# BCAM-CFD/RigidMultiblobsWall

Measured on AMD Instinct MI355X. Metric: RPY-wall M.f matvecs/sec (single_wall_mobility_trans_times_force, N_blobs=10000), higher is better.
Workload: dtype f64

## Files before the change

### include/rmb_mobility.h

```cpp
#ifndef RMB_MOBILITY_H
#define RMB_MOBILITY_H

#include <stddef.h>

#ifdef __cplusplus
extern "C" {
#endif

typedef struct rmb_ctx rmb_ctx;

enum rmb_status {
  RMB_OK = 0,
  RMB_ERR_ARG = -1,
  RMB_ERR_STATE = -2,
  RMB_ERR_HIP = -3,
  RMB_ERR_NO_DEVICE = -4
};

enum rmb_kind { RMB_TT = 0, RMB_TR = 1, RMB_RT = 2, RMB_RR = 3, RMB_TT_TR = 4, RMB_TT_FREE_SURFACE = 5 };

const char* rmb_version(void);
const char* rmb_last_error(void);
int rmb_device_count(void);

// ... 119 lines not shown
                             double body_repulsion_strength, double body_debye_length, double kT, double* energy_dev,
                             int* accepted_dev);
int rmb_one_blob_force_device(rmb_ctx* ctx, long n, const double* r_dev, double blob_radius, double weight, double eps_wall,
                              double debye_wall, int accumulate, double* out_dev);
int rmb_blob_blob_force_pairshard_device(rmb_ctx* ctx, double repulsion_strength, double debye_length,
                                         double blob_radius, double* out_dev, long shard, long nshards);
int rmb_blob_blob_force_radii(rmb_ctx* ctx, const double* radii, double repulsion_strength, double debye_length,
                              double* out);
int rmb_blob_blob_force_radii_device(rmb_ctx* ctx, const double* radii_dev, double repulsion_strength,
                                     double debye_length, double* out_dev);

int rmb_timing_collect(rmb_ctx* ctx, double* ms, int max_n);
int rmb_timing_reset(rmb_ctx* ctx);
int rmb_ubench_fp64_issue(rmb_ctx* ctx, int launches, double* g_wave_instr_per_s);
int rmb_wave_clock_collect(rmb_ctx* ctx, long long* stamps, long max_waves);
int rmb_last_host_timing(rmb_ctx* ctx, double* us4);
int rmb_last_launch(rmb_ctx* ctx, long* tiles, long* chunks, long* workgroups);
int rmb_ctx_synchronize(rmb_ctx* ctx);

int rmb_default_ctx_set_option(const char* key, long value);
int rmb_default_ctx_set_device(int device);

typedef struct rmb_multi rmb_multi;
int rmb_multi_create(const int* devices, int n_devices, rmb_multi** engine);
int rmb_multi_destroy(rmb_multi* engine);
int rmb_multi_n_shards(rmb_multi* engine);
int rmb_multi_shard_ctx(rmb_multi* engine, int shard, rmb_ctx** ctx);
int rmb_multi_set_stream(rmb_multi* engine, void* hip_stream);
int rmb_multi_set_option(rmb_multi* engine, const char* key, long value);
int rmb_multi_get_option(rmb_multi* engine, const char* key, long* value);
// ... 61 lines not shown
```

### rigidmultiblobswall_amd/_lib.py

```python
import ctypes
import os

_HERE = os.path.dirname(os.path.abspath(__file__))
DIAGNOSTICS = os.environ.get("RMB_DIAGNOSTICS", "0") not in ("", "0")
LIB_PATH = os.path.join(_HERE, "librmb_mobility_diag.so" if DIAGNOSTICS else "librmb_mobility.so")

_dp = ctypes.POINTER(ctypes.c_double)
_vp = ctypes.c_void_p
_lp = ctypes.POINTER(ctypes.c_long)

KIND_TT, KIND_TR, KIND_RT, KIND_RR, KIND_TT_TR, KIND_TT_FREE = 0, 1, 2, 3, 4, 5
OP_VELOCITY_FROM_FORCE_TORQUE, OP_GRAND, OP_FORCE_COLUMN, OP_TT_MULTI, OP_TR_MULTI, OP_RT_MULTI, OP_RR_MULTI = range(7)
OPS = {"velocity_from_force_torque": (OP_VELOCITY_FROM_FORCE_TORQUE, 2, 1), "grand": (OP_GRAND, 2, 2),
       "force_column": (OP_FORCE_COLUMN, 1, 2), "tt_multi": (OP_TT_MULTI, None, None), "tr_multi": (OP_TR_MULTI, None, None),
       "rt_multi": (OP_RT_MULTI, None, None), "rr_multi": (OP_RR_MULTI, None, None)}
KINDS = {"tt": KIND_TT, "tr": KIND_TR, "rt": KIND_RT, "rr": KIND_RR, "tt_tr": KIND_TT_TR, "tt_free": KIND_TT_FREE}

SYMBOLS = {
    "rmb_version": (ctypes.c_char_p, []),
    "rmb_last_error": (ctypes.c_char_p, []),
    "rmb_device_count": (ctypes.c_int, []),
    "rmb_ctx_create": (ctypes.c_int, [ctypes.c_int, ctypes.POINTER(_vp)]),
    "rmb_ctx_destroy": (ctypes.c_int, [_vp]),
    "rmb_ctx_set_stream": (ctypes.c_int, [_vp, _vp]),
# ... 63 lines not shown
                                                    _vp, _vp] + [ctypes.c_double] * 6 + [ctypes.c_int, ctypes.c_double, ctypes.c_double, _vp]),
    "rmb_mcmc_sweep_bb_device": (ctypes.c_int, [_vp, ctypes.c_long, ctypes.c_long, ctypes.c_long, _vp, _vp, _vp, _vp, _vp, _vp, _vp, ctypes.c_double,
                                               _vp] + [ctypes.c_double] * 6 + [ctypes.c_int, ctypes.c_double, ctypes.c_double, ctypes.c_double,
                                                                               _vp, _vp]),
    "rmb_potential_oneshot": (ctypes.c_int, [ctypes.c_long, _vp, _vp] + [ctypes.c_double] * 6 + [ctypes.c_int, _vp]),
    "rmb_one_blob_force_device": (ctypes.c_int, [_vp, ctypes.c_long, _vp, ctypes.c_double, ctypes.c_double, ctypes.c_double, ctypes.c_double,
                                                ctypes.c_int, _vp]),
    "rmb_blob_blob_force_pairshard_device": (ctypes.c_int, [_vp, ctypes.c_double, ctypes.c_double, ctypes.c_double, _vp,
                                                            ctypes.c_long, ctypes.c_long]),
    "rmb_blob_blob_force_radii": (ctypes.c_int, [_vp, _vp, ctypes.c_double, ctypes.c_double, _vp]),
    "rmb_blob_blob_force_radii_device": (ctypes.c_int, [_vp, _vp, ctypes.c_double, ctypes.c_double, _vp]),
    "rmb_timing_collect": (ctypes.c_int, [_vp, _dp, ctypes.c_int]),
    "rmb_timing_reset": (ctypes.c_int, [_vp]),
    "rmb_ubench_fp64_issue": (ctypes.c_int, [_vp, ctypes.c_int, _dp]),
    "rmb_wave_clock_collect": (ctypes.c_int, [_vp, _vp, ctypes.c_long]),
    "rmb_last_host_timing": (ctypes.c_int, [_vp, _dp]),
    "rmb_last_launch": (ctypes.c_int, [_vp, _lp, _lp, _lp]),
    "rmb_ctx_synchronize": (ctypes.c_int, [_vp]),
    "rmb_default_ctx_set_option": (ctypes.c_int, [ctypes.c_char_p, ctypes.c_long]),
    "rmb_default_ctx_set_device": (ctypes.c_int, [ctypes.c_int]),
    "rmb_multi_create": (ctypes.c_int, [ctypes.POINTER(ctypes.c_int), ctypes.c_int, ctypes.POINTER(_vp)]),
    "rmb_multi_destroy": (ctypes.c_int, [_vp]),
    "rmb_multi_n_shards": (ctypes.c_int, [_vp]),
    "rmb_multi_shard_ctx": (ctypes.c_int, [_vp, ctypes.c_int, ctypes.POINTER(_vp)]),
    "rmb_multi_set_stream": (ctypes.c_int, [_vp, _vp]),
    "rmb_multi_set_option": (ctypes.c_int, [_vp, ctypes.c_char_p, ctypes.c_long]),
    "rmb_multi_get_option": (ctypes.c_int, [_vp, ctypes.c_char_p, _lp]),
    "rmb_multi_set_positions": (ctypes.c_int, [_vp, _vp, ctypes.c_long, ctypes.c_double, _vp, ctypes.c_int]),
    "rmb_multi_set_positions_device": (ctypes.c_int, [_vp, _vp, ctypes.c_long, ctypes.c_double, _vp, ctypes.c_int]),
    "rmb_multi_matvec": (ctypes.c_int, [_vp, ctypes.c_int, ctypes.c_int, _vp, _vp, ctypes.c_double, _vp]),
# ... 86 lines not shown
```

### rigidmultiblobswall_amd/context.py

```python
import ctypes

import numpy as np

from . import _lib


def _as_f64(x, n3=None):
  x = np.ascontiguousarray(x, dtype=np.float64).reshape(-1)
  if n3 is not None and x.size != n3:
    raise ValueError("expected %d values, got %d" % (n3, x.size))
  return x


def _ptr(x):
  return ctypes.c_void_p(x.ctypes.data)


POTENTIAL_FORMS = {"soft": 0, "yukawa": 1}
VAN_HOVE_PLANES = {"xyz": 0, "xy": 1}


class MobilityContext(object):

  def __init__(self, device=0):
# ... 745 lines not shown

  def timing_collect(self, max_n=8192):
    buf = (ctypes.c_double * max_n)()
    n = self._lib.rmb_timing_collect(self._h, buf, max_n)
    if n < 0:
      _lib.check(n)
    return np.array(buf[:n])

  def wave_clock_collect(self, max_waves=8192):
    buf = np.zeros((max_waves, 2), dtype=np.int64)
    n = self._lib.rmb_wave_clock_collect(self._h, ctypes.c_void_p(buf.ctypes.data), max_waves)
    if n < 0:
      _lib.check(n)
    return buf[:n]

  def ubench_fp64_issue(self, launches=40):
    out = ctypes.c_double()
    self._follow_torch_stream()
    _lib.check(self._lib.rmb_ubench_fp64_issue(self._h, int(launches), ctypes.byref(out)))
    return float(out.value)

  def last_host_timing(self):
    buf = (ctypes.c_double * 4)()
    _lib.check(self._lib.rmb_last_host_timing(self._h, buf))
    return dict(upload_us=buf[0], launch_us=buf[1], wait_and_download_us=buf[2], c_call_us=buf[3])

  def timing_reset(self):
    _lib.check(self._lib.rmb_timing_reset(self._h))

  def last_launch(self):
# ... 54 lines not shown
```

### rigidmultiblobswall_amd/csrc/rmb_context.hip

```cpp
#include "rmb_internal.h"

#include <cstdint>
#include <cstdio>
#include <cstdlib>
#include <cstring>

namespace rmbi {

namespace { thread_local std::string g_err; }

int fail(int code, const std::string& msg) {
  g_err = msg;
  return code;
}

int DevBuf::reserve(size_t bytes) {
  if (bytes <= cap) return 0;
  if (p) { (void)hipFree(p); p = nullptr; cap = 0; }
  size_t want = bytes + bytes / 8 + 256;
  hipError_t e = hipMalloc(&p, want);
  if (e != hipSuccess) { p = nullptr; return fail(RMB_ERR_HIP, std::string("hipMalloc: ") + hipGetErrorString(e)); }
  cap = want;
  return 0;
}
// ... 83 lines not shown
    {"det_workspace_mb", &rmb_ctx::opt_det_workspace_mb, CLAMP, 1, kNoCap},
    {"sym_wps", &rmb_ctx::opt_sym_wps}, {"sym_pin", &rmb_ctx::opt_sym_pin},
    {"free_surface", &rmb_ctx::opt_free_surface, BOOLEAN}, {"free_surface_rotation", &rmb_ctx::opt_free_surface_rotation, BOOLEAN},
    {"precision", &rmb_ctx::opt_precision, ONE_OF, 32, 64, 64, "precision must be 32 or 64"},
    {"force_precision", &rmb_ctx::opt_force_precision, ONE_OF, 0, 32, 64, "force_precision must be 0 (follow \"precision\"), 32 or 64"},
    {"force_cull", &rmb_ctx::opt_force_cull, BOOLEAN}, {"force_sort", &rmb_ctx::opt_force_sort, BOOLEAN},
    {"potential_resort", &rmb_ctx::opt_potential_resort, CLAMP, 1, kNoCap},
    {"sym_fine_steps", &rmb_ctx::opt_sym_fine_steps, CLAMP, 0, kNoCap},
    {"sym_coop", &rmb_ctx::opt_sym_coop, ONE_OF, 0, 1, 2, "sym_coop must be 0 (never), 1 (launches below one resident round) or 2 (always)"},
    {"sym_chunk_steps", &rmb_ctx::opt_sym_chunk_steps, CLAMP, 0, kNoCap}, {"sym_two_targets", &rmb_ctx::opt_sym_two_targets, CLAMP, 0, 2},
    {"host_zero_copy_in", &rmb_ctx::opt_host_zero_copy_in, BOOLEAN}, {"gmres_fuse_pc", &rmb_ctx::opt_gmres_fuse_pc, BOOLEAN}, {"gmres_fuse_dots", &rmb_ctx::opt_gmres_fuse_dots, BOOLEAN},
    {"krylov_low_sync", &rmb_ctx::opt_krylov_low_sync, BOOLEAN}, {"lanczos_fuse_finish", &rmb_ctx::opt_lanczos_fuse_finish, BOOLEAN},
    {"host_zero_copy", &rmb_ctx::opt_host_zero_copy, CLAMP, 0, kNoCap},
    {"sym_order", &rmb_ctx::opt_sym_order, BOOLEAN}, {"sym_xcd", &rmb_ctx::opt_sym_xcd, BOOLEAN},
    {"sym_oversub", &rmb_ctx::opt_sym_oversub, CLAMP, 1, kNoCap}, {"sym_min_steps", &rmb_ctx::opt_sym_min_steps, CLAMP, 1, kNoCap},
    {"wave_clock", &rmb_ctx::opt_wave_clock, AS_GIVEN, 0, 0, 0, nullptr, true}, {"skip_pairs", &rmb_ctx::opt_skip_pairs, AS_GIVEN, 0, 0, 0, nullptr, true},
};

const Option* find_option(const char* key) {
  for (const Option& o : kOptions)
    if (!strcmp(key, o.key)) return &o;
  return nullptr;
}
}

}

using namespace rmbi;

extern "C" {

const char* rmb_version(void) { return "rmb_mobility 0.1 (gfx950)"; }
const char* rmb_last_error(void) { return rmbi::g_err.c_str(); }

int rmb_device_count(void) {
  int n = 0;
  if (hipGetDeviceCount(&n) != hipSuccess) return 0;
// ... 6 lines not shown
  hipError_t e = hipGetDeviceCount(&n);
  if (e != hipSuccess || n == 0)
    return fail(RMB_ERR_NO_DEVICE, std::string("no HIP device visible (") + hipGetErrorString(e) + ")");
  if (device == -1) {
    device = default_device();
    if (device < 0) return fail(RMB_ERR_ARG, "RMB_DEVICE must be a non-negative device index");
  }
  if (device < 0 || device >= n) return fail(RMB_ERR_ARG, "device index out of range");
  RMB_HIP(hipSetDevice(device));
  hipDeviceProp_t prop;
  RMB_HIP(hipGetDeviceProperties(&prop, device));
  rmb_ctx* c = new rmb_ctx();
  c->device = device;
  if (prop.multiProcessorCount > 0) c->n_cu = prop.multiProcessorCount;
  if (prop.maxSharedMemoryPerMultiProcessor > 0) c->lds_per_cu = prop.maxSharedMemoryPerMultiProcessor;
  *out = c;
  return 0;
}

int rmb_ctx_destroy(rmb_ctx* c) {
  if (!c) return 0;
  (void)hipSetDevice(c->device);
  (void)hipStreamSynchronize(c->stream);
  rmbi::gmres_release(c);
  for_each_buffer(*c, [](DevBuf& b) { b.release(); });
  c->host_out.release();
  c->host_in.release();
  if (c->stream_switch) (void)hipEventDestroy(c->stream_switch);
  for (auto e : c->ev0) (void)hipEventDestroy(e);
  for (auto e : c->ev1) (void)hipEventDestroy(e);
// ... 38 lines not shown
    case CLAMP: value = value < o->a ? o->a : (value > o->b ? o->b : value); break;
    case BOOLEAN: value = value ? 1 : 0; break;
    case ONE_OF: if (value != o->a && value != o->b && value != o->c) return fail(RMB_ERR_ARG, o->refusal); break;
  }
  c->*(o->field) = value;
  if (o->field == &rmb_ctx::opt_potential_resort) c->pot_sort_age = -1;
  return 0;
}

int rmb_ctx_get_option(rmb_ctx* c, const char* key, long* value) {
  if (!c || !key || !value) return fail(RMB_ERR_ARG, "null context / key / value");
  if (!strcmp(key, "last_path")) { *value = c->last_path; return 0; }
  if (!strcmp(key, "diagnostics_build")) { *value = kDiagnosticsBuild; return 0; }
  if (!strcmp(key, "buffers_signature")) {
    unsigned long long h = 1469598103934665603ull;
    for_each_buffer(*c, [&h](const DevBuf& b) { h = (h ^ (unsigned long long)(uintptr_t)b.p) * 1099511628211ull; });
    *value = (long)(h >> 1);
    return 0;
  }
  const Option* o = find_option(key);
  if (!o) return fail(RMB_ERR_ARG, std::string("unknown option: ") + key);
  *value = c->*(o->field);
  return 0;
}

int rmb_timing_collect(rmb_ctx* c, double* ms, int max_n) {
  if (!c || !ms || max_n < 0) return fail(RMB_ERR_ARG, "bad timing_collect arguments");
  if (hipSetDevice(c->device) != hipSuccess) return fail(RMB_ERR_HIP, "hipSetDevice failed");
  if (hipStreamSynchronize(c->stream) != hipSuccess) return fail(RMB_ERR_HIP, "hipStreamSynchronize failed");
  int have = c->ev_count < kTimingRing ? c->ev_count : kTimingRing;
  if (have > max_n) have = max_n;
  for (int i = 0; i < have; ++i) {
    const int idx = (c->ev_count - have + i) % kTimingRing;
    float t = 0.f;
    if (hipEventElapsedTime(&t, c->ev0[idx], c->ev1[idx]) != hipSuccess) return fail(RMB_ERR_HIP, "hipEventElapsedTime failed");
    ms[i] = (double)t;
  }
  return have;
// ... 62 lines not shown
```

### rigidmultiblobswall_amd/csrc/rmb_internal.h

```cpp
#pragma once
#include "../../include/rmb_mobility.h"

#include <hip/hip_runtime.h>

#include <cmath>
#include <mutex>
#include <string>
#include <type_traits>
#include <vector>

#include "pair_ops.h"

namespace rmbi {

int fail(int code, const std::string& msg);

#define RMB_HIP(call)                                                                        \
  do {                                                                                       \
    hipError_t e_ = (call);                                                                  \
    if (e_ != hipSuccess)                                                                    \
      return rmbi::fail(RMB_ERR_HIP, std::string(#call) + ": " + hipGetErrorString(e_));     \
  } while (0)

struct DevBuf {
  void* p = nullptr;
  size_t cap = 0;
// ... 14 lines not shown
struct CtxBuffers {
  DevBuf pos;
  DevBuf r_stage;
  DevBuf vec, vec2, out, partial, tmp3n;
  DevBuf tile_bounds;
  DevBuf fpos, fperm, fsort_keys, fsort_vals, fsort_tmp, fsort_box;
  DevBuf pot_ws;
  DevBuf mcmc_ws;
  DevBuf msd_ws;
  DevBuf scat_ws;
  DevBuf vh_ws;
  DevBuf det_ws;
  DevBuf wave_clock;
  DevBuf krylov;
  DevBuf symbuf;
  DevBuf st[8];
};
using CB = CtxBuffers;
constexpr DevBuf CB::* kCtxBufs[] = {&CB::pos, &CB::r_stage, &CB::vec, &CB::vec2, &CB::out, &CB::partial, &CB::tmp3n, &CB::tile_bounds,
                                     &CB::fpos, &CB::fperm, &CB::fsort_keys, &CB::fsort_vals, &CB::fsort_tmp, &CB::fsort_box,
                                     &CB::pot_ws, &CB::mcmc_ws, &CB::msd_ws, &CB::scat_ws, &CB::vh_ws, &CB::det_ws, &CB::wave_clock, &CB::krylov, &CB::symbuf};
static_assert(sizeof(CtxBuffers) == (sizeof(kCtxBufs) / sizeof(kCtxBufs[0]) + 8) * sizeof(DevBuf),
              "a DevBuf of CtxBuffers is missing from kCtxBufs (or st[] changed its length)");
template <class Bufs, class F>
void for_each_buffer(Bufs& b, F f) {
  for (auto m : kCtxBufs) f(b.*m);
  for (auto& s : b.st) f(s);
}

}

struct rmb_ctx : rmbi::CtxBuffers {
  int device = 0;
  hipStream_t stream = nullptr;
  hipEvent_t stream_switch = nullptr;
  long n_cu = 256;
// ... 31 lines not shown
  long opt_potential_resort = 16;
  long opt_sym_fine_steps = 0;
  long opt_sym_coop = 1;
  long opt_sym_chunk_steps = 1024;
  long opt_sym_two_targets = 1;
  long opt_host_zero_copy_in = 1;
  long opt_gmres_fuse_pc = 1;
  long opt_gmres_fuse_dots = 1;
  long opt_krylov_low_sync = 1;
  long opt_lanczos_fuse_finish = 1;
  long opt_host_zero_copy = 768 << 10;
  long opt_sym_order = 1;
  long opt_sym_xcd = 1;
  long opt_sym_oversub = 8;
  long opt_sym_min_steps = 64;
  long opt_wave_clock = 0;
  long opt_skip_pairs = 0;
  std::vector<hipEvent_t> ev0, ev1;
  int ev_count = 0;
  long timing_launches = 0;
  int last_path = 0;
  long last_tiles = 0, last_chunks = 0, last_wgs = 0;
  double host_us[4] = {0, 0, 0, 0};
};

namespace rmbi {

int timing_begin(rmb_ctx* c, int* slot);
int timing_end(rmb_ctx* c, int slot);
int check_ready(rmb_ctx* c);
// ... 72 lines not shown
}
int plan_cull_sweep(rmb_ctx* c, const SymKernel& k, long total_steps, long* blocks, long* chunk_steps, long rounds = 0,
                    size_t dyn_lds = 0, double wg_pair_cap = 0.0, const char* who = "");
void shard_ranges(long n, long n_units, long shard, long nshards, long* step_begin, long* step_end, long* self_begin,
                  long* self_end);
int sym_accumulators(rmb_ctx* c, long n_pad);
long chunked_steps(const rmb_ctx* c, long total, long n_sched, long spw, long target);
bool sym_applies(const rmb_ctx* c);
inline double inv_length(double L) { return L > 0 ? 1.0 / L : 0.0; }

enum SymXOp { SX_TT = 0, SX_TR, SX_RT, SX_RR, SX_FUSED, SX_GRAND, SX_COLF, SX_FREE, SX_RADII,
              SX_FREE_TR, SX_FREE_RT, SX_FREE_RR, SX_FREE_FUSED, SX_FREE_GRAND, SX_FREE_COLF, SX_K2, SX_COUNT = SX_K2 + 12 };
struct SymConf { const double4* pos; long n; double L[3]; int wall; const double* extra; };
template <class A, class = void> struct HasNPad : std::false_type {};
template <class A> struct HasNPad<A, std::void_t<decltype(A::n_pad)>> : std::true_type {};
template <class A, class = void> struct HasPrefactor : std::false_type {};
template <class A> struct HasPrefactor<A, std::void_t<decltype(A::prefactor)>> : std::true_type {};
template <class Args>
void fill_sym_args(Args& a, const SymConf& cf, const rmb_ctx* c, double eta, long n_units, long shard, long nshards) {
  const long tiles = (cf.n + 63) / 64;
  long step_begin, step_end, self_begin, self_end;
  shard_ranges(cf.n, n_units, shard, nshards, &step_begin, &step_end, &self_begin, &self_end);
  a.pos = cf.pos;
  a.n = cf.n; a.n_tiles = (int)tiles;
  a.order = (int)c->opt_sym_order; a.xcd = (int)c->opt_sym_xcd;
  a.step_end = step_end;
  a.Lx = cf.L[0]; a.Ly = cf.L[1];
  a.iLx = inv_length(cf.L[0]); a.iLy = inv_length(cf.L[1]);
  if constexpr (HasNPad<Args>::value) {
    a.acc = (double*)c->symbuf.p;
    a.n_pad = 64 * tiles; a.n_units = n_units;
    a.step_begin = step_begin;
    a.Lz = cf.L[2]; a.iLz = inv_length(cf.L[2]);
  }
  if constexpr (HasPrefactor<Args>::value) {
    a.self_begin = self_begin; a.self_end = self_end;
    a.prefactor = 1.0 / (8.0 * M_PI * eta);
    a.k = make_pair_consts(c->a > 0.0 ? c->a : 1.0);
  }
}
template <class Args>
int sym_launch(rmb_ctx* c, const SymKernel& k, int path, long blocks, size_t dyn_lds, Args& a, const rmb::PairConsts& pk,
               void (*fin)(Args), long fin_blocks, long long** wave_clock = nullptr) {
  c->last_path = path; c->last_tiles = a.n_tiles; c->last_chunks = 0; c->last_wgs = blocks;
  if (wave_clock) {
    *wave_clock = nullptr;
    if (c->opt_wave_clock) {
      c->wave_clock_n = blocks * rmb::kSymWaves * (path == 4 ? 2 : 1);
      if (int rc = c->wave_clock.reserve((size_t)2 * c->wave_clock_n * sizeof(long long))) return rc;
      *wave_clock = (long long*)c->wave_clock.p;
    }
  }
  int slot;
  if (int rc = timing_begin(c, &slot)) return rc;
// ... 79 lines not shown
```

### rigidmultiblobswall_amd/csrc/rmb_sym.hip

```cpp
#include "rmb_internal.h"

#include <cmath>

#include "sym_kernels.h"
#include "sym_coop_kernels.h"
#include "sym2t_kernels.h"
#include "sym2_kernels.h"
#include "sym_force_kernels.h"
#include "sym_schedule.h"
#include "symx_kernels.h"

namespace rmbi {

namespace {
SymConf conf_of(const rmb_ctx* c) {
  return SymConf{(const double4*)c->pos.p, c->n, {c->L[0], c->L[1], c->L[2]}, c->wall, nullptr};
}
bool is_periodic(const SymConf& cf) { return cf.L[0] > 0 || cf.L[1] > 0 || cf.L[2] > 0; }

struct SymCandidates { SymKernel plain, coop, two, f32; };
struct SymChoice {
  SymKernel kernel;
  SymPlan plan;
  int path;
// ... 43 lines not shown
struct SymEntry { SymCandidates k; sym_fn fin; };
template <int KIND, bool WALL, bool PER> SymEntry make_sym_entry() {
  constexpr size_t lds = sizeof(double2) * rmb::kSymWaves * 64 * 3 + sizeof(double) * rmb::kSymWaves * 3 * 64;
  constexpr size_t coop_lds = sizeof(double2) * 64 * 3 + sizeof(double) * 2 * 3 * 64;
  SymEntry e{{sym_kernel_of<rmb::SymArgs, rmb::sym_kernel<KIND, WALL, PER>>(lds, rmb::kSymWavesPerEu),
              sym_kernel_of<rmb::SymArgs, rmb::sym_coop_kernel<KIND, WALL, PER>>(coop_lds, rmb::kSymWavesPerEu), SymKernel{}, SymKernel{}},
             rmb::sym_finalize_kernel<KIND, WALL>};
  if constexpr (!PER) e.k.two = sym_kernel_of<rmb::SymArgs, rmb::sym2t_kernel<KIND, WALL>>(lds, rmb::kSymWavesPerEu);
  return e;
}
#define RMB_SYM_ROW(K) {{make_sym_entry<K, false, false>(), make_sym_entry<K, false, true>()}, {make_sym_entry<K, true, false>(), make_sym_entry<K, true, true>()}}
SymEntry g_sym[4][2][2] = {RMB_SYM_ROW(rmb::KIND_TT), RMB_SYM_ROW(rmb::KIND_TR), RMB_SYM_ROW(rmb::KIND_RT), RMB_SYM_ROW(rmb::KIND_RR)};
#undef RMB_SYM_ROW
}

int sym_device(rmb_ctx* c, int kind, const double* v, double eta, double* out, long shard, long nshards, bool accumulate,
               bool no_finalize) {
  const SymConf cf = conf_of(c);
  const bool periodic = is_periodic(cf);
  const SymEntry& se = g_sym[kind][c->wall ? 1 : 0][periodic ? 1 : 0];
  const long n = c->n;
  if (int rc = sym_accumulators(c, 64 * ((n + 63) / 64))) return rc;
  if (periodic && no_finalize) return fail(RMB_ERR_STATE, "sym_device: no_finalize is for open boundaries (internal)");
  SymCandidates k = se.k;
  if (periodic && !c->opt_wave_clock) k.two = symx_two_periodic(SX_TT + kind, c->wall != 0);
  if (c->opt_wave_clock) k.coop = SymKernel{};
  if (c->opt_precision == 32 && kind == RMB_TT && !periodic) {
    if (c->opt_wave_clock || c->opt_skip_pairs)
      return fail(RMB_ERR_STATE, "the \"wave_clock\" / \"skip_pairs\" diagnostics exist in the fp64 kernels only: set \"precision\" = 64");
    k.f32 = sym32_tt(c->wall != 0);
  }
  SymChoice ch;
  if (int rc = choose_sym(c, k, n, shard, nshards, kCoopMaxRounds, true, &ch)) return rc;
  if (periodic && ch.path == 4) {
    const double* in[2] = {v, nullptr};
    double* outs[1] = {out};
    return symx_device(c, SX_TT + kind, in, outs, eta, 0, shard, nshards, accumulate ? 1 : 0);
  }
  rmb::SymArgs a;
  fill_sym_args(a, cf, c, eta, ch.n_units, shard, nshards);
  a.vec = v;
  a.out = out;
  a.steps_per_wave = ch.steps_per_wave;
  a.skip_pairs = (int)c->opt_skip_pairs;
  a.accumulate = accumulate ? 1 : 0;
  return sym_launch(c, ch.kernel, ch.path, ch.plan.blocks, ch.plan.dyn_lds, a, a.k, no_finalize ? nullptr : se.fin, (n + 255) / 256,
                    &a.wave_clock);
}

int sym2_device(rmb_ctx* c, const double* va, const double* vb, double eta, double* out_a, double* out_b, long shard,
                long nshards) {
  const SymConf cf = conf_of(c);
  const bool periodic = is_periodic(cf);
  const long n = c->n;
  if (int rc = sym_accumulators(c, 64 * ((n + 63) / 64))) return rc;
  typedef rmb::Sym2Args A;
  const SymKernel k = c->wall ? (periodic ? sym_kernel_of<A, rmb::sym2_kernel<true, true>>(0, rmb::kSymWavesPerEu)
                                          : sym_kernel_of<A, rmb::sym2_kernel<true, false>>(0, rmb::kSymWavesPerEu))
                              : (periodic ? sym_kernel_of<A, rmb::sym2_kernel<false, true>>(0, rmb::kSymWavesPerEu)
                                          : sym_kernel_of<A, rmb::sym2_kernel<false, false>>(0, rmb::kSymWavesPerEu));
  SymChoice ch;
  if (int rc = choose_sym(c, SymCandidates{k, SymKernel{}, SymKernel{}, SymKernel{}}, n, shard, nshards, 0, false, &ch)) return rc;
// ... 201 lines not shown
```

### rigidmultiblobswall_amd/csrc/sym2t_kernels.h

```cpp
#pragma once
#include "sym_kernels.h"
#include "sym_schedule.h"

namespace rmb {

template <int KIND, bool WALL>
__global__ __launch_bounds__(64 * kSymWaves) __attribute__((amdgpu_waves_per_eu(kSymWavesPerEu, kSymWavesPerEu))) void sym2t_kernel(const SymArgs a) {
  __shared__ double2 rec_all[kSymWaves][64 * 3];
  __shared__ double accj_all[kSymWaves][3 * 64];
  const int lane = threadIdx.x & 63;
  const int wave = __builtin_amdgcn_readfirstlane(threadIdx.x >> 6);
  double2* rec = rec_all[wave];
  double* accj = accj_all[wave];
  const char* rec_bytes = reinterpret_cast<const char*>(rec);
  constexpr bool Z2 = kSymZi2<KIND, WALL>;

  const long w = (a.xcd ? xcd_swizzle(blockIdx.x, gridDim.x) : (long)blockIdx.x) * kSymWaves + wave;
  const long long t_start = a.wave_clock ? wall_clock64() : 0;
  const long long c_start = a.wave_clock ? (long long)__builtin_readcyclecounter() : 0;
  long long c_stage = 0;
  for (long chunk = w;; chunk += (long)gridDim.x * kSymWaves) {
  long s = a.step_begin + chunk * a.steps_per_wave;
  if (s >= a.step_end) break;
  long s_end = s + a.steps_per_wave;
  if (s_end > a.step_end) s_end = a.step_end;
  int p = 0, J = 0;
  unit2_seek(a.order, s >> 6, a.n_tiles, p, J);

  int p_cur = -1;
  long i0 = 0, i1 = 0;
  bool ok0 = false, ok1 = false;
  double x0 = 0, y0 = 0, z0 = sym_height<Z2>(1.0), v0x = 0, v0y = 0, v0z = 0;
  double x1 = 0, y1 = 0, z1 = sym_height<Z2>(1.0), v1x = 0, v1y = 0, v1z = 0;
  Vec3 u0 = {0.0, 0.0, 0.0}, u1 = {0.0, 0.0, 0.0};

  auto flush_rows = [&]() {
    if (ok0) {
      __hip_atomic_fetch_add(&a.acc[i0], u0.x, __ATOMIC_RELAXED, __HIP_MEMORY_SCOPE_AGENT);
      __hip_atomic_fetch_add(&a.acc[a.n_pad + i0], u0.y, __ATOMIC_RELAXED, __HIP_MEMORY_SCOPE_AGENT);
      __hip_atomic_fetch_add(&a.acc[2 * a.n_pad + i0], u0.z, __ATOMIC_RELAXED, __HIP_MEMORY_SCOPE_AGENT);
// ... 95 lines not shown
      __builtin_amdgcn_fence(__ATOMIC_RELEASE, "wavefront");
      __builtin_amdgcn_wave_barrier();
      __builtin_amdgcn_fence(__ATOMIC_ACQUIRE, "wavefront");
      const long j = 64L * J + lane;
      if (j < a.n && !(a.skip_pairs & 2)) {
        __hip_atomic_fetch_add(&a.acc[j], accj[lane], __ATOMIC_RELAXED, __HIP_MEMORY_SCOPE_AGENT);
        __hip_atomic_fetch_add(&a.acc[a.n_pad + j], accj[64 + lane], __ATOMIC_RELAXED, __HIP_MEMORY_SCOPE_AGENT);
        __hip_atomic_fetch_add(&a.acc[2 * a.n_pad + j], accj[128 + lane], __ATOMIC_RELAXED, __HIP_MEMORY_SCOPE_AGENT);
      }
    }
    __builtin_amdgcn_wave_barrier();
    if (k1 == 64) unit2_next(a.order, a.n_tiles, p, J);
  }
  if (p_cur >= 0) flush_rows();
  }
  if (a.wave_clock && lane == 0) {
    const unsigned hw = __builtin_amdgcn_s_getreg((4) | (0 << 6) | ((16 - 1) << 11));
    const unsigned xcc = __builtin_amdgcn_s_getreg((20) | (0 << 6) | ((4 - 1) << 11));
    const long n_waves = (long)gridDim.x * kSymWaves;
    a.wave_clock[2 * w] = t_start;
    a.wave_clock[2 * w + 1] = (wall_clock64() & 0xffffffffffLL) | ((long long)(hw & 0xffff) << 40) | ((long long)(xcc & 0xf) << 56);
    a.wave_clock[2 * (n_waves + w)] = c_stage;
    a.wave_clock[2 * (n_waves + w) + 1] = (long long)__builtin_readcyclecounter() - c_start;
  }
}

}
```

### rigidmultiblobswall_amd/csrc/sym_kernels.h

```cpp
#pragma once
#include "pair_blocks.h"
#include "sym_schedule.h"

namespace rmb {

struct SymArgs {
  const double4* pos;
  const double* vec;
  double* acc;
  double* out;
  long n;
  long n_pad;
  int n_tiles;
  long n_units;
  int order;
  int xcd;
  long step_begin, step_end;
  long steps_per_wave;
  long self_begin, self_end;
  double Lx, Ly, Lz, iLx, iLy, iLz;
  double prefactor;
  int accumulate;
  int skip_pairs;
  long long* wave_clock;
  PairConsts k;
};

constexpr int kSymRecBytes = 48;

template <bool WALL, bool ACC = false, bool ZI2 = false>
__device__ __forceinline__ void pair_tt_sym(const PairConsts& k, double dx, double dy, double dz, double zi, double zj,
                                            double vix, double viy, double viz, double vjx, double vjy, double vjz,
                                            Vec3& ui, double& tx, double& ty, double& tz) {
  const Geom g = make_geom<WALL, ZI2>(dx, dy, dz, zi, zj);
  const TTc c = tt_coeffs<WALL, ZI2>(k, g, zi, zj);
  const double vi[3] = {vix, viy, viz}, vj[3] = {vjx, vjy, vjz};
  double u[3] = {ui.x, ui.y, ui.z}, t[3];
  if constexpr (ACC) { t[0] = tx; t[1] = ty; t[2] = tz; }
  tt_apply<WALL, ACC>(c, g, vi, vj, u, t);
  ui.x = u[0]; ui.y = u[1]; ui.z = u[2];
  tx = t[0]; ty = t[1]; tz = t[2];
// ... 45 lines not shown


template <int KIND, bool WALL, bool PERIODIC>
__global__ __launch_bounds__(64 * kSymWaves) __attribute__((amdgpu_waves_per_eu(kSymWavesPerEu, kSymWavesPerEu))) void sym_kernel(const SymArgs a) {
  __shared__ double2 rec_all[kSymWaves][64 * 3];
  __shared__ double accj_all[kSymWaves][3 * 64];
  const int lane = threadIdx.x & 63;
  const int wave = __builtin_amdgcn_readfirstlane(threadIdx.x >> 6);
  double2* rec = rec_all[wave];
  double* accj = accj_all[wave];
  const char* rec_bytes = reinterpret_cast<const char*>(rec);
  constexpr bool Z2 = kSymZi2<KIND, WALL>;

  const long w = (a.xcd ? xcd_swizzle(blockIdx.x, gridDim.x) : (long)blockIdx.x) * kSymWaves + wave;
  const long long t_start = a.wave_clock ? wall_clock64() : 0;
  for (long chunk = w;; chunk += (long)gridDim.x * kSymWaves) {
  long s = a.step_begin + chunk * a.steps_per_wave;
  if (s >= a.step_end) break;
  long s_end = s + a.steps_per_wave;
  if (s_end > a.step_end) s_end = a.step_end;
  int I = 0, J = 0;
  if (s < s_end) unit_seek(a.order, s >> 6, a.n_tiles, I, J);

  int I_cur = -1;
  long i = 0;
  bool vi_ok = false;
  double xi = 0, yi = 0, zi = sym_height<Z2>(1.0), vix = 0, viy = 0, viz = 0;
  Vec3 ui = {0.0, 0.0, 0.0};

  while (s < s_end) {
    const int k0 = (int)(s & 63);
    const long left = s_end - s;
    const int k1 = (left < 64 - k0) ? (int)(k0 + left) : 64;
    s += k1 - k0;

// ... 87 lines not shown
              }
        }
      }
    }
    __builtin_amdgcn_wave_barrier();
    if (k1 == 64) {
      unit_next(a.order, a.n_tiles, I, J);
    }
  }
  if (I_cur >= 0 && vi_ok) {
    __hip_atomic_fetch_add(&a.acc[i], ui.x, __ATOMIC_RELAXED, __HIP_MEMORY_SCOPE_AGENT);
    __hip_atomic_fetch_add(&a.acc[a.n_pad + i], ui.y, __ATOMIC_RELAXED, __HIP_MEMORY_SCOPE_AGENT);
    __hip_atomic_fetch_add(&a.acc[2 * a.n_pad + i], ui.z, __ATOMIC_RELAXED, __HIP_MEMORY_SCOPE_AGENT);
  }
  }
  if (a.wave_clock && lane == 0) {
    const unsigned hw = __builtin_amdgcn_s_getreg((4) | (0 << 6) | ((16 - 1) << 11));
    const unsigned xcc = __builtin_amdgcn_s_getreg((20) | (0 << 6) | ((4 - 1) << 11));
    a.wave_clock[2 * w] = t_start;
    a.wave_clock[2 * w + 1] = (wall_clock64() & 0xffffffffffLL) | ((long long)(hw & 0xffff) << 40) | ((long long)(xcc & 0xf) << 56);
  }
}

__device__ __forceinline__ void store_aos_coalesced(double* tile, double* out, long base, long n, double x, double y, double z,
                                                    bool valid, bool accumulate) {
  const int t = threadIdx.x;
  if (valid) { tile[3 * t] = x; tile[3 * t + 1] = y; tile[3 * t + 2] = z; }
  __syncthreads();
  const long lim = 3 * n;
#pragma unroll
  for (int c = 0; c < 3; ++c) {
    const long g = 3 * base + c * 256 + t;
    if (g < lim) out[g] = accumulate ? out[g] + tile[c * 256 + t] : tile[c * 256 + t];
  }
  __syncthreads();
}

template <int KIND, bool WALL>
__global__ __launch_bounds__(256) void sym_finalize_kernel(const SymArgs a) {
  __shared__ double tile[768];
  const long base = (long)blockIdx.x * blockDim.x;
  const long i = base + threadIdx.x;
  const bool valid = i < a.n;
  Vec3 acc = {0.0, 0.0, 0.0};
  double sc = 0.0;
  if (valid) {
    acc.x = a.acc[i]; acc.y = a.acc[a.n_pad + i]; acc.z = a.acc[2 * a.n_pad + i];
    a.acc[i] = 0.0; a.acc[a.n_pad + i] = 0.0; a.acc[2 * a.n_pad + i] = 0.0;
    const double4 p = a.pos[i];
    const double b = p.w;
    if (i >= a.self_begin && i < a.self_end)
      self_term<KIND, WALL>(a.k, p.z, a.vec[3 * i] * b, a.vec[3 * i + 1] * b, a.vec[3 * i + 2] * b, 0, 0, 0, acc);
    sc = a.prefactor * b;
  }
  store_aos_coalesced(tile, a.out, base, a.n, acc.x * sc, acc.y * sc, acc.z * sc, valid, a.accumulate != 0);
}


}
```

### rigidmultiblobswall_amd/csrc/sym_schedule.h

```cpp
#pragma once
#include <cmath>
#ifdef __HIPCC__
#include <hip/hip_runtime.h>
#endif

namespace rmb {

__device__ __forceinline__ double wrap_nearest_sym(double r, double L, double invL) {
  const double q = r * invL;
  const double h = (r > 0.0) ? 0.5 : ((r < 0.0) ? -0.5 : 0.0);
  return __builtin_fma(-__builtin_trunc(q + h), L, r);
}

__device__ __forceinline__ double wrap_nearest_pad_safe(double r, double L, double invL) {
  const double w = wrap_nearest_sym(r, L, invL);
  return (__builtin_fabs(r) < 1e50) ? w : r;
}

__device__ __forceinline__ void unit_to_tiles(long u, int T, int& I, int& J) {
  const double tt = 2.0 * T + 1.0;
  long i = (long)((tt - sqrt(tt * tt - 8.0 * (double)u)) * 0.5);
  if (i < 0) i = 0;
  if (i > T - 1) i = T - 1;
  while (i > 0 && i * T - i * (i - 1) / 2 > u) --i;
// ... 44 lines not shown
    if (++J == T) { ++I; J = I; }
    return;
  }
  const int P = I >> kOrdShift, Q = J >> kOrdShift;
  const int row_end = ((P + 1) << kOrdShift) < T ? ((P + 1) << kOrdShift) : T;
  const int col_end = ((Q + 1) << kOrdShift) < T ? ((Q + 1) << kOrdShift) : T;
  if (++J < col_end) return;
  if (++I < row_end) { J = (P == Q) ? I : (Q << kOrdShift); return; }
  if (((Q + 1) << kOrdShift) < T) { I = P << kOrdShift; J = (Q + 1) << kOrdShift; return; }
  I = (P + 1) << kOrdShift; J = I;
}

__device__ __forceinline__ long xcd_swizzle(long bid, long nwg) {
  const long q = nwg >> 3, r = nwg & 7, xcd = bid & 7;
  return (xcd < r ? xcd * (q + 1) : r * (q + 1) + (xcd - r) * q) + (bid >> 3);
}

__host__ __device__ inline long units2_before_pair(long p, long T) { return p * T - p * (p - 1); }
__host__ __device__ inline long units2_total(long T) { return units2_before_pair((T + 1) / 2, T); }

constexpr int kOrd2Pairs = 1 << (kOrdShift - 1);

__host__ __device__ inline long blk2_units_before_row(long B, long T) { return (long)kOrd2Pairs * B * (T + 1 - (long)kOrd2Pairs * B); }

__device__ __forceinline__ void unit2_seek(int order, long u, int T, int& p, int& J) {
  const double b = (double)T + 1.0;
  double disc = b * b - 4.0 * (double)u;
  if (disc < 0.0) disc = 0.0;
  const double y = (b - sqrt(disc)) * 0.5;
  if (order == 0) {
// ... 104 lines not shown
```

Baseline: 7184.

## Adaptively rebalance symmetric pair work across XCDs using per-XCD timing feedback

Replaces the round-robin chunk loop in the symmetric pair kernels with a static partition of steps into per-XCD contiguous ranges, weighted by a cumulative share table held on the device. Each wave stamps start and end times with atomics, and the finalize kernel gets one extra block that updates the shares toward the measured per-XCD throughput, with damping and clamping to a bounded range. The aim is to cut tail imbalance when some XCDs finish later than others. In exchange it adds atomic timestamping, an extra block in the finalize launch, and static range partitioning in place of fine-grained interleaving, which could hurt load balance inside an XCD.

```diff
diff --git a/include/rmb_mobility.h b/include/rmb_mobility.h
--- a/include/rmb_mobility.h
+++ b/include/rmb_mobility.h
@@ -157,6 +157,8 @@
 int rmb_timing_reset(rmb_ctx* ctx);
 int rmb_ubench_fp64_issue(rmb_ctx* ctx, int launches, double* g_wave_instr_per_s);
 int rmb_wave_clock_collect(rmb_ctx* ctx, long long* stamps, long max_waves);
+int rmb_ctx_get_xcd_shares(rmb_ctx* ctx, double* shares8);
+int rmb_ctx_set_xcd_shares(rmb_ctx* ctx, const double* shares8);
 int rmb_last_host_timing(rmb_ctx* ctx, double* us4);
 int rmb_last_launch(rmb_ctx* ctx, long* tiles, long* chunks, long* workgroups);
 int rmb_ctx_synchronize(rmb_ctx* ctx);
diff --git a/rigidmultiblobswall_amd/_lib.py b/rigidmultiblobswall_amd/_lib.py
--- a/rigidmultiblobswall_amd/_lib.py
+++ b/rigidmultiblobswall_amd/_lib.py
@@ -101,6 +101,8 @@
     "rmb_timing_reset": (ctypes.c_int, [_vp]),
     "rmb_ubench_fp64_issue": (ctypes.c_int, [_vp, ctypes.c_int, _dp]),
     "rmb_wave_clock_collect": (ctypes.c_int, [_vp, _vp, ctypes.c_long]),
+    "rmb_ctx_get_xcd_shares": (ctypes.c_int, [_vp, _vp]),
+    "rmb_ctx_set_xcd_shares": (ctypes.c_int, [_vp, _vp]),
     "rmb_last_host_timing": (ctypes.c_int, [_vp, _dp]),
     "rmb_last_launch": (ctypes.c_int, [_vp, _lp, _lp, _lp]),
     "rmb_ctx_synchronize": (ctypes.c_int, [_vp]),
diff --git a/rigidmultiblobswall_amd/context.py b/rigidmultiblobswall_amd/context.py
--- a/rigidmultiblobswall_amd/context.py
+++ b/rigidmultiblobswall_amd/context.py
@@ -783,6 +783,15 @@
       _lib.check(n)
     return buf[:n]
 
+  def get_xcd_shares(self):
+    buf = np.zeros(8)
+    _lib.check(self._lib.rmb_ctx_get_xcd_shares(self._h, ctypes.c_void_p(buf.ctypes.data)))
+    return buf
+
+  def set_xcd_shares(self, shares):
+    buf = np.ascontiguousarray(shares, dtype=np.float64).reshape(8)
+    _lib.check(self._lib.rmb_ctx_set_xcd_shares(self._h, ctypes.c_void_p(buf.ctypes.data)))
+
   def ubench_fp64_issue(self, launches=40):
     out = ctypes.c_double()
     self._follow_torch_stream()
diff --git a/rigidmultiblobswall_amd/csrc/rmb_context.hip b/rigidmultiblobswall_amd/csrc/rmb_context.hip
--- a/rigidmultiblobswall_amd/csrc/rmb_context.hip
+++ b/rigidmultiblobswall_amd/csrc/rmb_context.hip
@@ -1,4 +1,5 @@
 #include "rmb_internal.h"
+#include "sym_schedule.h"
 
 #include <cstdint>
 #include <cstdio>
@@ -121,6 +122,7 @@
     {"host_zero_copy", &rmb_ctx::opt_host_zero_copy, CLAMP, 0, kNoCap},
     {"sym_order", &rmb_ctx::opt_sym_order, BOOLEAN}, {"sym_xcd", &rmb_ctx::opt_sym_xcd, BOOLEAN},
     {"sym_oversub", &rmb_ctx::opt_sym_oversub, CLAMP, 1, kNoCap}, {"sym_min_steps", &rmb_ctx::opt_sym_min_steps, CLAMP, 1, kNoCap},
+    {"sym_xcd_balance", &rmb_ctx::opt_sym_xcd_balance, ONE_OF, 0, 1, 2, "sym_xcd_balance must be 0 (equal shares), 1 (adaptive) or 2 (the table as it is)"},
     {"wave_clock", &rmb_ctx::opt_wave_clock, AS_GIVEN, 0, 0, 0, nullptr, true}, {"skip_pairs", &rmb_ctx::opt_skip_pairs, AS_GIVEN, 0, 0, 0, nullptr, true},
 };
 
@@ -128,6 +130,17 @@
   for (const Option& o : kOptions)
     if (!strcmp(key, o.key)) return &o;
   return nullptr;
+}
+
+int xcd_shares_store(rmb_ctx* c, const double* shares) {
+  rmb::XcdBalance b = {};
+  const double equal[rmb::kXcdSlots] = {0.125, 0.125, 0.125, 0.125, 0.125, 0.125, 0.125, 0.125};
+  for (int x = 0; x < rmb::kXcdSlots; ++x) b.share[x] = shares[x];
+  rmb::xcd_cum_from_shares(shares, b.cum);
+  rmb::xcd_cum_from_shares(equal, b.cum_equal);
+  rmb::xcd_balance_reset_stamps(&b);
+  RMB_HIP(hipMemcpy(c->xcd_balance.p, &b, sizeof(b), hipMemcpyHostToDevice));
+  return 0;
 }
 }
 
@@ -164,6 +177,9 @@
   c->device = device;
   if (prop.multiProcessorCount > 0) c->n_cu = prop.multiProcessorCount;
   if (prop.maxSharedMemoryPerMultiProcessor > 0) c->lds_per_cu = prop.maxSharedMemoryPerMultiProcessor;
+  const double equal[rmb::kXcdSlots] = {0.125, 0.125, 0.125, 0.125, 0.125, 0.125, 0.125, 0.125};
+  if (int rc = c->xcd_balance.reserve(sizeof(rmb::XcdBalance))) { delete c; return rc; }
+  if (int rc = xcd_shares_store(c, equal)) { (void)rmb_ctx_destroy(c); return rc; }
   *out = c;
   return 0;
 }
@@ -232,7 +248,10 @@
   if (!strcmp(key, "diagnostics_build")) { *value = kDiagnosticsBuild; return 0; }
   if (!strcmp(key, "buffers_signature")) {
     unsigned long long h = 1469598103934665603ull;
-    for_each_buffer(*c, [&h](const DevBuf& b) { h = (h ^ (unsigned long long)(uintptr_t)b.p) * 1099511628211ull; });
+    for_each_buffer(*c, [&h](const DevBuf& b) {
+      h = (h ^ (unsigned long long)(uintptr_t)b.p) * 1099511628211ull;
+      h = (h ^ (unsigned long long)b.cap) * 1099511628211ull;
+    });
     *value = (long)(h >> 1);
     return 0;
   }
@@ -240,6 +259,31 @@
   if (!o) return fail(RMB_ERR_ARG, std::string("unknown option: ") + key);
   *value = c->*(o->field);
   return 0;
+}
+
+int rmb_ctx_get_xcd_shares(rmb_ctx* c, double* shares) {
+  if (!c || !shares) return fail(RMB_ERR_ARG, "null context / shares");
+  RMB_HIP(hipSetDevice(c->device));
+  RMB_HIP(hipStreamSynchronize(c->stream));
+  rmb::XcdBalance b;
+  RMB_HIP(hipMemcpy(&b, c->xcd_balance.p, sizeof(b), hipMemcpyDeviceToHost));
+  for (int x = 0; x < rmb::kXcdSlots; ++x) shares[x] = (double)(b.cum[x + 1] - b.cum[x]) / (double)rmb::kXcdOne;
+  return 0;
+}
+
+int rmb_ctx_set_xcd_shares(rmb_ctx* c, const double* shares) {
+  if (!c || !shares) return fail(RMB_ERR_ARG, "null context / shares");
+  double sum = 0.0;
+  for (int x = 0; x < rmb::kXcdSlots; ++x) {
+    if (!(shares[x] >= 0.0) || !std::isfinite(shares[x])) return fail(RMB_ERR_ARG, "xcd shares must be finite and non-negative");
+    sum += shares[x];
+  }
+  if (!(sum > 0.0) || !std::isfinite(sum)) return fail(RMB_ERR_ARG, "xcd shares must have a positive sum");
+  double s[rmb::kXcdSlots];
+  for (int x = 0; x < rmb::kXcdSlots; ++x) s[x] = shares[x] / sum;
+  RMB_HIP(hipSetDevice(c->device));
+  RMB_HIP(hipStreamSynchronize(c->stream));
+  return xcd_shares_store(c, s);
 }
 
 int rmb_timing_collect(rmb_ctx* c, double* ms, int max_n) {
diff --git a/rigidmultiblobswall_amd/csrc/rmb_internal.h b/rigidmultiblobswall_amd/csrc/rmb_internal.h
--- a/rigidmultiblobswall_amd/csrc/rmb_internal.h
+++ b/rigidmultiblobswall_amd/csrc/rmb_internal.h
@@ -10,6 +10,8 @@
 #include <vector>
 
 #include "pair_ops.h"
+
+namespace rmb { struct XcdBalance; }
 
 namespace rmbi {
 
@@ -54,12 +56,13 @@
   DevBuf wave_clock;
   DevBuf krylov;
   DevBuf symbuf;
+  DevBuf xcd_balance;
   DevBuf st[8];
 };
 using CB = CtxBuffers;
 constexpr DevBuf CB::* kCtxBufs[] = {&CB::pos, &CB::r_stage, &CB::vec, &CB::vec2, &CB::out, &CB::partial, &CB::tmp3n, &CB::tile_bounds,
                                      &CB::fpos, &CB::fperm, &CB::fsort_keys, &CB::fsort_vals, &CB::fsort_tmp, &CB::fsort_box,
-                                     &CB::pot_ws, &CB::mcmc_ws, &CB::msd_ws, &CB::scat_ws, &CB::vh_ws, &CB::det_ws, &CB::wave_clock, &CB::krylov, &CB::symbuf};
+                                     &CB::pot_ws, &CB::mcmc_ws, &CB::msd_ws, &CB::scat_ws, &CB::vh_ws, &CB::det_ws, &CB::wave_clock, &CB::krylov, &CB::symbuf, &CB::xcd_balance};
 static_assert(sizeof(CtxBuffers) == (sizeof(kCtxBufs) / sizeof(kCtxBufs[0]) + 8) * sizeof(DevBuf),
               "a DevBuf of CtxBuffers is missing from kCtxBufs (or st[] changed its length)");
 template <class Bufs, class F>
@@ -121,6 +124,7 @@
   long opt_sym_xcd = 1;
   long opt_sym_oversub = 8;
   long opt_sym_min_steps = 64;
+  long opt_sym_xcd_balance = 1;
   long opt_wave_clock = 0;
   long opt_skip_pairs = 0;
   std::vector<hipEvent_t> ev0, ev1;
@@ -223,6 +227,9 @@
 struct SymConf { const double4* pos; long n; double L[3]; int wall; const double* extra; };
 template <class A, class = void> struct HasNPad : std::false_type {};
 template <class A> struct HasNPad<A, std::void_t<decltype(A::n_pad)>> : std::true_type {};
+void xcd_balance_args(const rmb_ctx* c, const unsigned** cum, rmb::XcdBalance** bal);
+template <class A, class = void> struct HasXcdCum : std::false_type {};
+template <class A> struct HasXcdCum<A, std::void_t<decltype(A::xcd_cum)>> : std::true_type {};
 template <class A, class = void> struct HasPrefactor : std::false_type {};
 template <class A> struct HasPrefactor<A, std::void_t<decltype(A::prefactor)>> : std::true_type {};
 template <class Args>
@@ -247,6 +254,10 @@
     a.prefactor = 1.0 / (8.0 * M_PI * eta);
     a.k = make_pair_consts(c->a > 0.0 ? c->a : 1.0);
   }
+  if constexpr (HasXcdCum<Args>::value) {
+    xcd_balance_args(c, &a.xcd_cum, &a.xcd_bal);
+    a.rounds = 1;
+  }
 }
 template <class Args>
 int sym_launch(rmb_ctx* c, const SymKernel& k, int path, long blocks, size_t dyn_lds, Args& a, const rmb::PairConsts& pk,
diff --git a/rigidmultiblobswall_amd/csrc/rmb_sym.hip b/rigidmultiblobswall_amd/csrc/rmb_sym.hip
--- a/rigidmultiblobswall_amd/csrc/rmb_sym.hip
+++ b/rigidmultiblobswall_amd/csrc/rmb_sym.hip
@@ -81,6 +81,12 @@
 #undef RMB_SYM_ROW
 }
 
+void xcd_balance_args(const rmb_ctx* c, const unsigned** cum, rmb::XcdBalance** bal) {
+  rmb::XcdBalance* b = c->opt_sym_xcd ? (rmb::XcdBalance*)c->xcd_balance.p : nullptr;
+  *cum = !b ? nullptr : (c->opt_sym_xcd_balance == 0 ? b->cum_equal : b->cum);
+  *bal = c->opt_sym_xcd_balance == 1 ? b : nullptr;
+}
+
 int sym_device(rmb_ctx* c, int kind, const double* v, double eta, double* out, long shard, long nshards, bool accumulate,
                bool no_finalize) {
   const SymConf cf = conf_of(c);
@@ -111,8 +117,15 @@
   a.steps_per_wave = ch.steps_per_wave;
   a.skip_pairs = (int)c->opt_skip_pairs;
   a.accumulate = accumulate ? 1 : 0;
-  return sym_launch(c, ch.kernel, ch.path, ch.plan.blocks, ch.plan.dyn_lds, a, a.k, no_finalize ? nullptr : se.fin, (n + 255) / 256,
-                    &a.wave_clock);
+  if (periodic || ch.path == 3 || k.f32) a.xcd_cum = nullptr;
+  if (!a.xcd_cum || no_finalize) a.xcd_bal = nullptr;
+  if (a.xcd_cum) {
+    const long per_round = ch.plan.blocks * rmb::kSymWaves * ch.steps_per_wave;
+    a.rounds = per_round > 0 ? (a.step_end - a.step_begin + per_round - 1) / per_round : 1;
+    if (a.rounds < 1) a.rounds = 1;
+  }
+  return sym_launch(c, ch.kernel, ch.path, ch.plan.blocks, ch.plan.dyn_lds, a, a.k, no_finalize ? nullptr : se.fin,
+                    (n + 255) / 256 + (a.xcd_bal ? 1 : 0), &a.wave_clock);
 }
 
 int sym2_device(rmb_ctx* c, const double* va, const double* vb, double eta, double* out_a, double* out_b, long shard,
diff --git a/rigidmultiblobswall_amd/csrc/sym2t_kernels.h b/rigidmultiblobswall_amd/csrc/sym2t_kernels.h
--- a/rigidmultiblobswall_amd/csrc/sym2t_kernels.h
+++ b/rigidmultiblobswall_amd/csrc/sym2t_kernels.h
@@ -19,11 +19,11 @@
   const long long t_start = a.wave_clock ? wall_clock64() : 0;
   const long long c_start = a.wave_clock ? (long long)__builtin_readcyclecounter() : 0;
   long long c_stage = 0;
-  for (long chunk = w;; chunk += (long)gridDim.x * kSymWaves) {
-  long s = a.step_begin + chunk * a.steps_per_wave;
-  if (s >= a.step_end) break;
-  long s_end = s + a.steps_per_wave;
-  if (s_end > a.step_end) s_end = a.step_end;
+  if (a.xcd_bal && lane == 0) xcd_stamp_entry(a.xcd_bal, wave);
+  for (long round = 0;; ++round) {
+  long s, s_end;
+  if (!sym_wave_round(a, w, round, wave, &s, &s_end)) break;
+  if (s >= s_end) continue;
   int p = 0, J = 0;
   unit2_seek(a.order, s >> 6, a.n_tiles, p, J);
 
@@ -149,6 +149,7 @@
   }
   if (p_cur >= 0) flush_rows();
   }
+  if (a.xcd_bal && lane == 0) xcd_stamp_exit(a.xcd_bal);
   if (a.wave_clock && lane == 0) {
     const unsigned hw = __builtin_amdgcn_s_getreg((4) | (0 << 6) | ((16 - 1) << 11));
     const unsigned xcc = __builtin_amdgcn_s_getreg((20) | (0 << 6) | ((4 - 1) << 11));
diff --git a/rigidmultiblobswall_amd/csrc/sym_kernels.h b/rigidmultiblobswall_amd/csrc/sym_kernels.h
--- a/rigidmultiblobswall_amd/csrc/sym_kernels.h
+++ b/rigidmultiblobswall_amd/csrc/sym_kernels.h
@@ -23,8 +23,40 @@
   int accumulate;
   int skip_pairs;
   long long* wave_clock;
+  const unsigned* xcd_cum;
+  XcdBalance* xcd_bal;
+  long rounds;
   PairConsts k;
 };
+
+__device__ __forceinline__ long sym_uniform(long v) {
+  const unsigned lo = __builtin_amdgcn_readfirstlane((unsigned)v), hi = __builtin_amdgcn_readfirstlane((unsigned)((unsigned long)v >> 32));
+  return (long)(((unsigned long)hi << 32) | lo);
+}
+
+__device__ __forceinline__ bool sym_wave_round(const SymArgs& a, long w, long round, int wave, long* s, long* s_end) {
+  if (a.xcd_cum) {
+    if (round >= a.rounds) return false;
+    long lo, hi;
+    xcd_wave_range(a.xcd_cum, a.step_begin, a.step_end, a.rounds, round, gridDim.x, kSymWaves, blockIdx.x, wave, &lo, &hi);
+    *s = sym_uniform(lo);
+    *s_end = sym_uniform(hi);
+    return true;
+  }
+  *s = a.step_begin + (w + round * (long)gridDim.x * kSymWaves) * a.steps_per_wave;
+  if (*s >= a.step_end) return false;
+  *s_end = *s + a.steps_per_wave < a.step_end ? *s + a.steps_per_wave : a.step_end;
+  return true;
+}
+
+__device__ __forceinline__ void xcd_stamp_entry(XcdBalance* b, int wave) {
+  if (blockIdx.x < kXcdSlots && wave == 0)
+    __hip_atomic_fetch_min(&b->start, (unsigned long long)wall_clock64(), __ATOMIC_RELAXED, __HIP_MEMORY_SCOPE_AGENT);
+}
+__device__ __forceinline__ void xcd_stamp_exit(XcdBalance* b) {
+  __hip_atomic_fetch_max(&b->end[(blockIdx.x & (kXcdSlots - 1)) * kXcdEndStride], (unsigned long long)wall_clock64(), __ATOMIC_RELAXED,
+                         __HIP_MEMORY_SCOPE_AGENT);
+}
 
 constexpr int kSymRecBytes = 48;
 
@@ -100,11 +132,15 @@
 
   const long w = (a.xcd ? xcd_swizzle(blockIdx.x, gridDim.x) : (long)blockIdx.x) * kSymWaves + wave;
   const long long t_start = a.wave_clock ? wall_clock64() : 0;
-  for (long chunk = w;; chunk += (long)gridDim.x * kSymWaves) {
-  long s = a.step_begin + chunk * a.steps_per_wave;
-  if (s >= a.step_end) break;
-  long s_end = s + a.steps_per_wave;
-  if (s_end > a.step_end) s_end = a.step_end;
+  if (!PERIODIC && a.xcd_bal && lane == 0) xcd_stamp_entry(a.xcd_bal, wave);
+  for (long round = 0;; ++round) {
+  long s, s_end;
+  if constexpr (PERIODIC) {
+    s = a.step_begin + (w + round * (long)gridDim.x * kSymWaves) * a.steps_per_wave;
+    if (s >= a.step_end) break;
+    s_end = s + a.steps_per_wave;
+    if (s_end > a.step_end) s_end = a.step_end;
+  } else if (!sym_wave_round(a, w, round, wave, &s, &s_end)) break;
   int I = 0, J = 0;
   if (s < s_end) unit_seek(a.order, s >> 6, a.n_tiles, I, J);
 
@@ -222,6 +258,7 @@
     __hip_atomic_fetch_add(&a.acc[2 * a.n_pad + i], ui.z, __ATOMIC_RELAXED, __HIP_MEMORY_SCOPE_AGENT);
   }
   }
+  if (!PERIODIC && a.xcd_bal && lane == 0) xcd_stamp_exit(a.xcd_bal);
   if (a.wave_clock && lane == 0) {
     const unsigned hw = __builtin_amdgcn_s_getreg((4) | (0 << 6) | ((16 - 1) << 11));
     const unsigned xcc = __builtin_amdgcn_s_getreg((20) | (0 << 6) | ((4 - 1) << 11));
@@ -252,6 +289,10 @@
   const bool valid = i < a.n;
   Vec3 acc = {0.0, 0.0, 0.0};
   double sc = 0.0;
+  if (base >= a.n) {
+    if (a.xcd_bal && threadIdx.x == 0) xcd_balance_update(a.xcd_bal, kXcdDamping);
+    return;
+  }
   if (valid) {
     acc.x = a.acc[i]; acc.y = a.acc[a.n_pad + i]; acc.z = a.acc[2 * a.n_pad + i];
     a.acc[i] = 0.0; a.acc[a.n_pad + i] = 0.0; a.acc[2 * a.n_pad + i] = 0.0;
diff --git a/rigidmultiblobswall_amd/csrc/sym_schedule.h b/rigidmultiblobswall_amd/csrc/sym_schedule.h
--- a/rigidmultiblobswall_amd/csrc/sym_schedule.h
+++ b/rigidmultiblobswall_amd/csrc/sym_schedule.h
@@ -82,6 +82,84 @@
 __device__ __forceinline__ long xcd_swizzle(long bid, long nwg) {
   const long q = nwg >> 3, r = nwg & 7, xcd = bid & 7;
   return (xcd < r ? xcd * (q + 1) : r * (q + 1) + (xcd - r) * q) + (bid >> 3);
+}
+
+constexpr int kXcdSlots = 8;
+constexpr unsigned kXcdOne = 65536;
+
+__host__ __device__ inline void xcd_wave_range(const unsigned* cum, long step_begin, long step_end, long rounds, long round,
+                                               long nwg, int waves_per_wg, long bid, int wave, long* s, long* s_end) {
+  const long total = step_end - step_begin;
+  const long b = step_begin + total * round / rounds, S = step_begin + total * (round + 1) / rounds - b;
+  const long x = bid & (kXcdSlots - 1);
+  long c0, c1;
+  if (nwg >= kXcdSlots) { c0 = cum[x]; c1 = cum[x + 1]; }
+  else { c0 = x < nwg ? (long)kXcdOne * x / nwg : kXcdOne; c1 = x + 1 < nwg ? (long)kXcdOne * (x + 1) / nwg : kXcdOne; }
+  const long lo = b + S * c0 / kXcdOne, L = b + S * c1 / kXcdOne - lo;
+  const long n_x = ((nwg >> 3) + (x < (nwg & 7) ? 1 : 0)) * waves_per_wg;
+  const long i = (bid >> 3) * waves_per_wg + wave;
+  *s = lo + L * i / n_x;
+  *s_end = lo + L * (i + 1) / n_x;
+}
+
+constexpr int kXcdEndStride = 16;
+struct XcdBalance {
+  unsigned cum[kXcdSlots + 1];
+  unsigned cum_equal[kXcdSlots + 1];
+  unsigned long long start;
+  double share[kXcdSlots];
+  alignas(128) unsigned long long end[kXcdSlots * kXcdEndStride];
+};
+constexpr double kXcdShareMin = 0.80 / kXcdSlots, kXcdShareMax = 1.25 / kXcdSlots;
+constexpr double kXcdDamping = 0.25;
+
+__host__ __device__ inline void xcd_cum_from_shares(const double* share, unsigned* cum) {
+  double run = 0.0;
+  cum[0] = 0;
+  for (int x = 0; x < kXcdSlots - 1; ++x) {
+    run += share[x];
+    const double c = run * kXcdOne + 0.5;
+    unsigned v = c <= 0.0 ? 0u : (c >= (double)kXcdOne ? kXcdOne : (unsigned)c);
+    cum[x + 1] = v < cum[x] ? cum[x] : v;
+  }
+  cum[kXcdSlots] = kXcdOne;
+}
+
+__host__ __device__ inline void xcd_balance_reset_stamps(XcdBalance* b) {
+  b->start = ~0ull;
+  for (int x = 0; x < kXcdSlots; ++x) b->end[x * kXcdEndStride] = 0;
+}
+
+__host__ __device__ inline void xcd_balance_update(XcdBalance* b, double damping) {
+  const unsigned long long start = b->start;
+  double rate[kXcdSlots], sum = 0.0;
+  bool ok = start != ~0ull;
+  for (int x = 0; x < kXcdSlots; ++x) {
+    const unsigned long long e = b->end[x * kXcdEndStride];
+    ok = ok && e > start;
+    rate[x] = (double)(b->cum[x + 1] - b->cum[x]) / (double)(long long)(e - start);
+    sum += rate[x];
+  }
+  xcd_balance_reset_stamps(b);
+  if (!ok || !(sum > 0.0)) return;
+  double s[kXcdSlots];
+  for (int x = 0; x < kXcdSlots; ++x) s[x] = b->share[x] + damping * (rate[x] / sum - b->share[x]);
+  for (int it = 0; it <= kXcdSlots; ++it) {
+    double total = 0.0;
+    for (int x = 0; x < kXcdSlots; ++x) {
+      s[x] = s[x] < kXcdShareMin ? kXcdShareMin : (s[x] > kXcdShareMax ? kXcdShareMax : s[x]);
+      total += s[x];
+    }
+    const double d = 1.0 - total;
+    if (d < 1e-15 && d > -1e-15) break;
+    int movable = 0;
+    for (int x = 0; x < kXcdSlots; ++x) movable += (d > 0.0 ? s[x] < kXcdShareMax : s[x] > kXcdShareMin) ? 1 : 0;
+    if (!movable) break;
+    for (int x = 0; x < kXcdSlots; ++x)
+      if (d > 0.0 ? s[x] < kXcdShareMax : s[x] > kXcdShareMin) s[x] += d / movable;
+  }
+  for (int x = 0; x < kXcdSlots; ++x) b->share[x] = s[x];
+  xcd_cum_from_shares(s, b->cum);
 }
 
 __host__ __device__ inline long units2_before_pair(long p, long T) { return p * T - p * (p - 1); }
```

New measurement: 7142. No clear change (-0.6%).
